# pixeli99/SVD_Xtend

Measured on NVIDIA H100. Metric: SVD UNet train-step frames/sec @ 14x320x512 bf16, higher is better.
Workload: dtype bf16

## Files before the change

include/svd_xtend_b200.h:

```cpp
#ifndef SVD_XTEND_B200_H_
#define SVD_XTEND_B200_H_

#include <stdint.h>

#ifdef __cplusplus
extern "C" {
#endif

#define SVDX_OK 0
#define SVDX_E_BADARG (-1)
#define SVDX_E_CUDA (-2)
#define SVDX_E_NODRIVER (-3)

#define SVDX_MAX_TAPS 27

#define SVDX_A_ROWS 0
#define SVDX_A_CONV2D 1

#define SVDX_OUT_BF16 0
#define SVDX_OUT_F32 1
#define SVDX_OUT_F32_ATOMIC 2

typedef struct SvdxTapGemm {
  const void* a;
// ... 23 lines not shown
  int64_t ldrb;
  const void* res1;
  int64_t ldr1;
  const void* res2;
  int64_t ldr2;
  const float* scales;
  void* pre;
  int64_t ldpre;
  float* gn_sum;
  int64_t gn_ld;
  int32_t gn_rows;
  const void* gnb_x;
  int64_t gnb_ldx;
  const void* gnb_x2;
  int64_t gnb_ldx2;
  int32_t gnb_c1;
  const float* gnb_ab;
  float* gnb_sum;
  int32_t gnb_rows;
  int32_t gnb_silu;
  int32_t interleave;
  int32_t phase_h, phase_w;
  int32_t act;
} SvdxTapGemm;

#define SVDX_ACT_NONE 0
#define SVDX_ACT_GELU 1
#define SVDX_ACT_QUICK_GELU 2

int svdx_tapgemm(const SvdxTapGemm* desc, void* stream);

int svdx_splitk_epilogue(float* ws, int64_t ldw, void* out, int64_t ldo, int64_t rows, int32_t cols, const float* bias,
                         const float* rowbias, int32_t rowbias_div, int64_t ldrb, const void* res1, int64_t ldr1,
                         const void* res2, int64_t ldr2, const float* scales, void* stream);

int svdx_num_sms(void);
int svdx_enable_peer_access(int32_t peer_device);
int svdx_ipc_export(const void* ptr, void* handle64_out, int64_t* offset_out);
int svdx_ipc_import(const void* handle64, int64_t offset, void** ptr_out);
int svdx_struct_size(int which);
const char* svdx_last_error(void);

int svdx_groupnorm_sums(const void* x, int64_t ldx, int32_t C1, const void* x2, int64_t ldx2, int32_t C2,
                        int32_t outer, int32_t rows, float* sums, int64_t ld, void* stream);
int svdx_groupnorm_apply_fused(const void* x, int64_t ldx, int32_t C1, const void* x2, int64_t ldx2, int32_t C2,
                               int32_t outer, int32_t rows, int32_t num_groups, float eps,
                               const float* csum1, int64_t ldc1, const float* csum2, int64_t ldc2,
                               float* mean, float* rstd, const float* gamma, const float* beta,
                               int32_t fuse_silu, void* y, int64_t ldy, float* ab_out, void* stream);
int svdx_groupnorm_bwd_sums(const void* x, int64_t ldx, int32_t C1, const void* x2, int64_t ldx2, int32_t C2,
                            const void* dy, int64_t lddy, int32_t outer, int32_t rows, const float* ab, int32_t fuse_silu,
// ... 146 lines not shown
```

svd_xtend_b200/_lib.py:

```python
from __future__ import annotations

import ctypes as C
import os
from pathlib import Path

PKG = Path(__file__).resolve().parent
LIB_PATH = Path(os.environ["SVDX_LIB"]) if os.environ.get("SVDX_LIB") else PKG / "lib" / "libsvdx_b200.so"

SVDX_MAX_TAPS = 27
SVDX_CLIP_MAX_TAPS = 63
A_ROWS, A_CONV2D = 0, 1
OUT_BF16, OUT_F32, OUT_F32_ATOMIC = 0, 1, 2
ACT_NONE, ACT_GELU, ACT_QUICK_GELU = 0, 1, 2

c_void_p, c_int, c_i64, c_float = C.c_void_p, C.c_int32, C.c_int64, C.c_float


class SvdxTapGemm(C.Structure):
    _fields_ = [
        ("a", c_void_p), ("lda", c_i64), ("a_mode", c_int), ("a_major_mn", c_int),
        ("rows_per_group", c_int), ("groups", c_int),
        ("W", c_int), ("H", c_int), ("nimg", c_int),
        ("num_taps", c_int),
        ("tap_d0", c_int * SVDX_MAX_TAPS), ("tap_d1", c_int * SVDX_MAX_TAPS), ("tap_d2", c_int * SVDX_MAX_TAPS),
        ("b", c_void_p), ("ldb", c_i64), ("b_major_mn", c_int), ("b_mode", c_int),
        ("M", c_int), ("N", c_int), ("K", c_int),
        ("block_n", c_int), ("split_k", c_int),
        ("out", c_void_p), ("ldo", c_i64), ("out_dtype", c_int), ("geglu", c_int),
        ("bias", c_void_p), ("rowbias", c_void_p), ("rowbias_div", c_int), ("ldrb", c_i64),
        ("res1", c_void_p), ("ldr1", c_i64), ("res2", c_void_p), ("ldr2", c_i64),
        ("scales", c_void_p), ("pre", c_void_p), ("ldpre", c_i64),
        ("gn_sum", c_void_p), ("gn_ld", c_i64), ("gn_rows", c_int),
        ("gnb_x", c_void_p), ("gnb_ldx", c_i64), ("gnb_x2", c_void_p), ("gnb_ldx2", c_i64), ("gnb_c1", c_int),
        ("gnb_ab", c_void_p), ("gnb_sum", c_void_p), ("gnb_rows", c_int), ("gnb_silu", c_int),
        ("interleave", c_int), ("phase_h", c_int), ("phase_w", c_int),
        ("act", c_int),
    ]


class SvdxAttn(C.Structure):
    _fields_ = [
        ("q", c_void_p), ("k", c_void_p), ("v", c_void_p), ("o", c_void_p),
        ("ldq", c_i64), ("ldk", c_i64), ("ldv", c_i64), ("ldo", c_i64),
        ("nseq", c_int), ("heads", c_int), ("S", c_int), ("inner", c_int),
        ("outer_stride", c_i64), ("inner_stride", c_i64), ("tok_stride", c_i64),
        ("scale", c_float), ("lse", c_void_p),
        ("dout", c_void_p), ("lddo", c_i64),
        ("dq", c_void_p), ("dk", c_void_p), ("dv", c_void_p),
        ("lddq", c_i64), ("lddk", c_i64), ("lddv", c_i64),
        ("delta", c_void_p),
    ]


_PROTOS = {
    "svdx_tapgemm": [C.POINTER(SvdxTapGemm), c_void_p],
    "svdx_splitk_epilogue": [c_void_p, c_i64, c_void_p, c_i64, c_i64, c_int, c_void_p, c_void_p, c_int, c_i64, c_void_p, c_i64,
                             c_void_p, c_i64, c_void_p, c_void_p],
    "svdx_num_sms": [],
    "svdx_enable_peer_access": [c_int],
# ... 126 lines not shown
```

svd_xtend_b200/csrc/common.cuh:

```cuda
#pragma once
#include <cuda.h>
#include <cuda_bf16.h>
#include <cuda_runtime.h>
#include <stdint.h>
#include <stdio.h>

#include "wgmma.cuh"

namespace svdx {

typedef __nv_bfloat16 bf16;

#define SVDX_DEVINL __device__ __forceinline__

#ifndef SVDX_WAIT_TIMEOUT_CYCLES
#define SVDX_WAIT_TIMEOUT_CYCLES (4000000000ll)
#endif

SVDX_DEVINL uint32_t smem_u32(const void* p) { return (uint32_t)__cvta_generic_to_shared(p); }

SVDX_DEVINL uint32_t lane_id() { return threadIdx.x & 31; }

SVDX_DEVINL bool elect_one() {
  uint32_t pred = 0;
// ... 93 lines not shown
               ::"l"(reinterpret_cast<uint64_t>(m)), "r"(src), "r"(c0), "r"(c1), "r"(c2)
               : "memory");
}
SVDX_DEVINL void bulk_commit() { asm volatile("cp.async.bulk.commit_group;" ::: "memory"); }
template <int N>
SVDX_DEVINL void bulk_wait_read() { asm volatile("cp.async.bulk.wait_group.read %0;" ::"n"(N) : "memory"); }
template <int N>
SVDX_DEVINL void bulk_wait() { asm volatile("cp.async.bulk.wait_group %0;" ::"n"(N) : "memory"); }
SVDX_DEVINL void st_shared_v4(uint32_t addr, uint32_t a, uint32_t b, uint32_t c, uint32_t d) {
  asm volatile("st.shared.v4.b32 [%0], {%1, %2, %3, %4};" ::"r"(addr), "r"(a), "r"(b), "r"(c), "r"(d) : "memory");
}

SVDX_DEVINL void wgmma_fence() { asm volatile("wgmma.fence.sync.aligned;" ::: "memory"); }
SVDX_DEVINL void wgmma_commit() { asm volatile("wgmma.commit_group.sync.aligned;" ::: "memory"); }
template <int N>
SVDX_DEVINL void wgmma_wait() { asm volatile("wgmma.wait_group.sync.aligned %0;" ::"n"(N) : "memory"); }
template <int R>
SVDX_DEVINL void reg_fence(float (&d)[R]) {
#pragma unroll
  for (int i = 0; i < R; ++i) asm volatile("" : "+f"(d[i])::"memory");
}

SVDX_DEVINL void named_bar_sync(int id, int nthreads) { asm volatile("bar.sync %0, %1;" ::"r"(id), "r"(nthreads) : "memory"); }

SVDX_DEVINL uint64_t make_smem_desc_sw128(uint32_t saddr, uint32_t lbo_bytes, uint32_t sbo_bytes) {
  uint64_t d = 0;
  d |= (uint64_t)((saddr & 0x3FFFF) >> 4);
  d |= (uint64_t)((lbo_bytes >> 4) & 0x3FFF) << 16;
  d |= (uint64_t)((sbo_bytes >> 4) & 0x3FFF) << 32;
  d |= (uint64_t)1 << 62;
  return d;
}

SVDX_DEVINL float silu_f(float x) { return __fdividef(x, 1.0f + __expf(-x)); }
SVDX_DEVINL float silu_grad_f(float x) {
  const float s = __fdividef(1.0f, 1.0f + __expf(-x));
  return s * fmaf(x, 1.0f - s, 1.0f);
}
#define SVDX_HDINL __host__ __device__ __forceinline__
SVDX_HDINL float gelu_tail_log2(float ax) {
  float p = -1.92123457e-06f;
  p = fmaf(p, ax, 6.32884985e-05f);
  p = fmaf(p, ax, -0.000943420862f);
  p = fmaf(p, ax, 0.0085562719f);
  p = fmaf(p, ax, -0.0540522821f);
  p = fmaf(p, ax, -0.458381772f);
// ... 45 lines not shown
```

svd_xtend_b200/csrc/tapgemm.cu:

```cuda
#include "tapgemm_common.cuh"

namespace svdx {

struct Ring {
  uint32_t sA, sB, bar_full, bar_empty;
  int stage;
  uint32_t phase;
};
template <int BN, int TA, int TB, int STG>
__device__ __forceinline__ void tile_mainloop(float (&acc)[BN / 2], int kb0, int kb1, Ring& rg, int wg) {
#pragma unroll
  for (int i = 0; i < BN / 2; ++i) acc[i] = 0.f;
  const int lane = threadIdx.x & 31;
  const uint32_t astep = TA ? (2048 >> 4) : (32 >> 4), bstep = TB ? (2048 >> 4) : (32 >> 4);
  int prev_stage = -1;
  for (int kb = kb0; kb < kb1; ++kb) {
    mbar_wait_mma(rg.bar_full + 8 * rg.stage, rg.phase);
    const uint32_t aaddr = rg.sA + rg.stage * A_STAGE_BYTES + wg * 8192;
    const uint32_t baddr = rg.sB + rg.stage * B_STAGE_BYTES;
    const uint64_t ad0 = make_smem_desc_sw128(aaddr, 8192, 1024);
    const uint64_t bd0 = make_smem_desc_sw128(baddr, 8192, 1024);
    wgmma_fence();
#pragma unroll
    for (int j = 0; j < BLOCK_K / 16; ++j) {
      const uint32_t accumulate = (kb > kb0 || j > 0) ? 1u : 0u;
      if constexpr (BN == 32) wgmma_ss_n32<TA, TB>(acc, ad0 + j * astep, bd0 + j * bstep, accumulate);
      else if constexpr (BN == 64) wgmma_ss_n64<TA, TB>(acc, ad0 + j * astep, bd0 + j * bstep, accumulate);
      else if constexpr (BN == 96) wgmma_ss_n96<TA, TB>(acc, ad0 + j * astep, bd0 + j * bstep, accumulate);
      else if constexpr (BN == 128) wgmma_ss_n128<TA, TB>(acc, ad0 + j * astep, bd0 + j * bstep, accumulate);
      else wgmma_ss_n160<TA, TB>(acc, ad0 + j * astep, bd0 + j * bstep, accumulate);
    }
    wgmma_commit();
    wgmma_wait<1>();
    reg_fence(acc);
    if (prev_stage >= 0) {
      __syncwarp();
      if (lane == 0) mbar_arrive(rg.bar_empty + 8 * prev_stage);
    }
    prev_stage = rg.stage;
    if (++rg.stage == STG) { rg.stage = 0; rg.phase ^= 1; }
  }
  wgmma_wait<0>();
  reg_fence(acc);
  __syncwarp();
  if (lane == 0 && prev_stage >= 0) mbar_arrive(rg.bar_empty + 8 * prev_stage);
}

template <int BN, int TA, int TB>
SVDX_DEVINL void tile_parked_bn(int kb0, int kb1, Ring& rg, uint32_t sAcc, int wg) {
  float acc[BN / 2];
  tile_mainloop<BN, TA, TB, STAGES_PARKED>(acc, kb0, kb1, rg, wg);
  const int lane = threadIdx.x & 31;
  const int r0 = wg * 64 + ((threadIdx.x >> 5) & 3) * 16 + (lane >> 2);
// ... 30 lines not shown
SVDX_DEVINL void tile_regs(const TapGemmKParams& p, int kb0, int kb1, Ring& rg, int wg, PairStage& ps, const EpiTile& t, int lane,
                           float s_acc, float s_r1, float s_r2) {
  if constexpr (EPI == EPI_GEGLU) {
    if (p.block_n == 64) tile_regs_bn<EPI, 64, 0>(p, kb0, kb1, rg, wg, ps, t, lane, s_acc, s_r1, s_r2);
    else tile_regs_bn<EPI, 128, 0>(p, kb0, kb1, rg, wg, ps, t, lane, s_acc, s_r1, s_r2);
  } else {
    if constexpr (EPI == EPI_FAST) {
      if (p.b_mn) {
        if (p.block_n == 64) tile_regs_bn<EPI, 64, 1>(p, kb0, kb1, rg, wg, ps, t, lane, s_acc, s_r1, s_r2);
        else tile_regs_bn<EPI, 128, 1>(p, kb0, kb1, rg, wg, ps, t, lane, s_acc, s_r1, s_r2);
        return;
      }
    }
    switch (p.block_n) {
      case 32: tile_regs_bn<EPI, 32, 0>(p, kb0, kb1, rg, wg, ps, t, lane, s_acc, s_r1, s_r2); break;
      case 64: tile_regs_bn<EPI, 64, 0>(p, kb0, kb1, rg, wg, ps, t, lane, s_acc, s_r1, s_r2); break;
      case 96: tile_regs_bn<EPI, 96, 0>(p, kb0, kb1, rg, wg, ps, t, lane, s_acc, s_r1, s_r2); break;
      case 128: tile_regs_bn<EPI, 128, 0>(p, kb0, kb1, rg, wg, ps, t, lane, s_acc, s_r1, s_r2); break;
      default: tile_regs_bn<EPI, 160, 0>(p, kb0, kb1, rg, wg, ps, t, lane, s_acc, s_r1, s_r2); break;
    }
  }
}

template <int BN, int TA, int TB>
SVDX_DEVINL void tile_f32_bn(const TapGemmKParams& p, int kb0, int kb1, Ring& rg, int wg, EpiStage& st, const EpiTile& t, int sub, int lane,
                             float s_acc) {
  float acc[BN / 2];
  tile_mainloop<BN, TA, TB, STAGES_REGS>(acc, kb0, kb1, rg, wg);
  epilogue_f32<BN>(p, acc, st, t, sub, lane, s_acc);
}

template <int TA>
SVDX_DEVINL void tile_f32(const TapGemmKParams& p, int kb0, int kb1, Ring& rg, int wg, EpiStage& st, const EpiTile& t, int sub, int lane,
                          float s_acc) {
  if (p.b_mn) {
    if (p.block_n == 64) tile_f32_bn<64, TA, 1>(p, kb0, kb1, rg, wg, st, t, sub, lane, s_acc);
    else tile_f32_bn<128, TA, 1>(p, kb0, kb1, rg, wg, st, t, sub, lane, s_acc);
    return;
  }
  switch (p.block_n) {
    case 32: tile_f32_bn<32, TA, 0>(p, kb0, kb1, rg, wg, st, t, sub, lane, s_acc); break;
    case 64: tile_f32_bn<64, TA, 0>(p, kb0, kb1, rg, wg, st, t, sub, lane, s_acc); break;
    case 96: tile_f32_bn<96, TA, 0>(p, kb0, kb1, rg, wg, st, t, sub, lane, s_acc); break;
    case 128: tile_f32_bn<128, TA, 0>(p, kb0, kb1, rg, wg, st, t, sub, lane, s_acc); break;
    default: tile_f32_bn<160, TA, 0>(p, kb0, kb1, rg, wg, st, t, sub, lane, s_acc); break;
  }
}

template <int EPI>
__global__ void __launch_bounds__(NUM_THREADS, 1) tapgemm_kernel(const __grid_constant__ TapGemmKParams p) {
  constexpr bool PARKED = EPI == EPI_GENERIC;
  constexpr int STAGES = PARKED ? STAGES_PARKED : STAGES_REGS;
  extern __shared__ uint8_t smem_raw[];
  const uint32_t smem_base = (smem_u32(smem_raw) + 1023u) & ~1023u;
  const uint32_t sA = smem_base;
  const uint32_t sB = smem_base + STAGES * A_STAGE_BYTES;
  const uint32_t sAcc = sB + STAGES * B_STAGE_BYTES;
  const uint32_t sEpi = sAcc + (PARKED ? ACC_BYTES : 0);
  const uint32_t sBar = sEpi + NUM_EPI_WARPS * EPI_STAGE_BYTES;
  const uint32_t bar_full = sBar;
  const uint32_t bar_empty = sBar + 8 * STAGES;

  const int warp = threadIdx.x >> 5;
  const int lane = threadIdx.x & 31;

  if (warp == PRODUCER_WARP && lane == 0) {
    prefetch_tmap(&p.tma);
    prefetch_tmap(&p.tmb);
    for (int i = 0; i < STAGES; ++i) {
      mbar_init(bar_full + 8 * i, 1);
      mbar_init(bar_empty + 8 * i, NUM_EPI_WARPS);
    }
    fence_barrier_init();
  }
  __syncthreads();

  const int total_tiles = p.m_tiles * p.n_tiles * p.split_k;
  const int b_bytes = p.block_n * BLOCK_K * 2;

  if (warp == PRODUCER_WARP) {
    const bool conv_par = (p.a_mode == SVDX_A_CONV2D) && !p.a_mn && !p.b_mn && !p.geglu && !p.wtiles && !p.im2col && (BLOCK_M / p.W) <= 32;
    if (conv_par) {
      int stage = 0;
      uint32_t phase = 0;
      for (int tile = blockIdx.x; tile < total_tiles; tile += gridDim.x) {
        const int nt = tile % p.n_tiles;
        const int mt = (tile / p.n_tiles) % p.m_tiles;
        const int ks = tile / (p.n_tiles * p.m_tiles);
        const int kb0 = ks * p.kb_per_split;
        const int kb1 = min(kb0 + p.kb_per_split, p.kb_total);
        const int n0 = nt * p.block_n;
        ConvBox bx;
        conv_tile_boxes(p, mt, lane, bx);
        const CUtensorMap* amap = bx.lg == 0 ? &p.tma : &p.tma_bh[bx.lg - 1];
        int tap = kb0 / p.kb_per_tap;
        int kci = kb0 - tap * p.kb_per_tap;
        for (int kb = kb0; kb < kb1; ++kb) {
          const uint32_t full = bar_full + 8 * stage;
          if (lane == 0) {
            mbar_wait_mma(bar_empty + 8 * stage, phase ^ 1);
            mbar_expect_tx(full, A_STAGE_BYTES + b_bytes);
// ... 138 lines not shown
                  tma_load_4d(&p.tmb, full, dB + j * 8192 + i * p.W * 128, n0 + 64 * j, dw, row - n * p.H + dh, nn);
                }
              }
            }
          } else if (p.b_mn && p.b_mode == 2) {
            const int g = kb / p.kb_per_group;
            const int k0 = (kb - g * p.kb_per_group) * BLOCK_K;
            for (int j = 0; j < p.block_n / 64; ++j)
              tma_load_3d(&p.tmb, full, dB + j * 8192, n0 + 64 * j, k0 + p.tap_d0[0], g);
          } else if (p.b_mn) {
            for (int j = 0; j < p.block_n / 64; ++j)
              tma_load_2d(&p.tmb, full, dB + j * 8192, n0 + 64 * j, kb * BLOCK_K);
          } else if (p.geglu) {
            const int h = p.block_n / 2;
            tma_load_2d(&p.tmb, full, dB, tap * p.K + kc, n0);
            tma_load_2d(&p.tmb, full, dB + h * 128, tap * p.K + kc, p.N / 2 + n0);
          } else {
            tma_load_2d(&p.tmb, full, dB, tap * p.K + kc, n0);
          }
          if (++stage == STAGES) { stage = 0; phase ^= 1; }
        }
      }
    }
  } else {
    const int wg = warp >> 2;
    const int q = PARKED ? (warp & 3) : (warp >> 1);
    const int half = PARKED ? (warp >> 2) : (warp & 1);
    Ring rg{sA, sB, bar_full, bar_empty, 0, 0u};
    float s_acc = 1.f, s_r1 = 1.f, s_r2 = 1.f;
    if (p.scales) { s_acc = p.scales[0]; s_r1 = p.scales[1]; s_r2 = p.scales[2]; }
    const int n_out_total = p.geglu ? p.N / 2 : p.N;
    const int bn_out = p.geglu ? p.block_n / 2 : p.block_n;
    EpiStage st;
    st.base = sEpi + warp * EPI_STAGE_BYTES;
    st.off = 0;
    PairStage ps{sEpi + q * 2 * EPI_STAGE_BYTES, 2 + q, half, 0u};
    const uint32_t t_base = sAcc + (uint32_t)((q * 32 + lane) * ACC_LD) * 4u;
    for (int tile = blockIdx.x; tile < total_tiles; tile += gridDim.x) {
      const int nt = tile % p.n_tiles;
      const int mt = (tile / p.n_tiles) % p.m_tiles;
      const int ks = tile / (p.n_tiles * p.m_tiles);
      const int kb0 = ks * p.kb_per_split;
      const int kb1 = min(kb0 + p.kb_per_split, p.kb_total);
      const int n0 = nt * bn_out;
      long long m;
      bool row_ok;
// ... 277 lines not shown
    if (d->act != SVDX_ACT_GELU && d->act != SVDX_ACT_QUICK_GELU) return svdx_fail(SVDX_E_BADARG, "tapgemm: act must be SVDX_ACT_GELU or SVDX_ACT_QUICK_GELU");
    if (p.epi_mode != EPI_FAST || p.rowbias || p.split_k > 1 || p.gn_sum)
      return svdx_fail(SVDX_E_BADARG, "tapgemm: act needs the plain bf16 TMA-store epilogue (bias only: no rowbias / residual / scales / "
                                      "GEGLU / split-K / gn_sum / gnb sums / interleave; N %% 32 == 0, aligned rows)");
    p.act = d->act;
    p.epi_mode = EPI_FAST_ACT;
  }
  if (d->b_major_mn && p.epi_mode != EPI_GENERIC && p.epi_mode != EPI_F32 && (p.epi_mode != EPI_FAST || p.gn_sum))
    return svdx_fail(SVDX_E_BADARG, "tapgemm: MN-major B takes the plain epilogue only (no gn_sum / gnb sums / act)");
  if (wide320 && p.epi_mode != EPI_FAST && p.epi_mode != EPI_RES && p.epi_mode != EPI_FAST_GNB && p.epi_mode != EPI_FAST_IL && p.epi_mode != EPI_FAST_ACT)
    return svdx_fail(SVDX_E_BADARG, "tapgemm: block_n 320 needs a bf16 output through the TMA-store epilogues (N % 320 == 0, aligned rows)");
  if (p.gn_sum) {
    if (p.epi_mode != EPI_FAST && p.epi_mode != EPI_RES && p.epi_mode != EPI_FAST_IL)
      return svdx_fail(SVDX_E_BADARG, "tapgemm: gn_sum needs a bf16 output through the TMA-store epilogues (N % 32 == 0, aligned rows), no split-K / GEGLU");
    if (p.gn_rows <= 0 || p.gn_ld < n_out || (p.gn_ld & 1) || (reinterpret_cast<uintptr_t>(p.gn_sum) & 7))
      return svdx_fail(SVDX_E_BADARG, "tapgemm: gn_sum needs gn_rows > 0, even gn_ld >= N, 8-byte aligned buffer");
  }
  if (d->out_dtype == SVDX_OUT_BF16 && ((d->ldo % 8) || (reinterpret_cast<uintptr_t>(d->out) & 15))) return svdx_fail(SVDX_E_BADARG, "tapgemm: out alignment");
  if (d->out_dtype != SVDX_OUT_BF16 && ((d->ldo % 4) || (reinterpret_cast<uintptr_t>(d->out) & 15))) return svdx_fail(SVDX_E_BADARG, "tapgemm: out alignment");
  if (d->res1 && ((d->ldr1 % 8) || (reinterpret_cast<uintptr_t>(d->res1) & 15))) return svdx_fail(SVDX_E_BADARG, "tapgemm: res1 alignment");
  if (d->res2 && ((d->ldr2 % 8) || (reinterpret_cast<uintptr_t>(d->res2) & 15))) return svdx_fail(SVDX_E_BADARG, "tapgemm: res2 alignment");
  if (d->pre && ((d->ldpre % 8) || (reinterpret_cast<uintptr_t>(d->pre) & 15))) return svdx_fail(SVDX_E_BADARG, "tapgemm: pre alignment");

  return SVDX_OK;
}

static constexpr int kernel_smem(int epi) { return epi == EPI_GENERIC ? smem_bytes(STAGES_PARKED, true) : smem_bytes(STAGES_REGS, false); }

template <int EPI>
static cudaError_t set_smem() {
  return cudaFuncSetAttribute(tapgemm_kernel<EPI>, cudaFuncAttributeMaxDynamicSharedMemorySize, kernel_smem(EPI));
}
template <int EPI>
static void launch(int grid, cudaStream_t stream, const TapGemmKParams& p) {
  tapgemm_kernel<EPI><<<grid, NUM_THREADS, kernel_smem(EPI), stream>>>(p);
}

extern "C" int svdx_tapgemm(const SvdxTapGemm* d, void* stream_v) {
  cudaStream_t stream = reinterpret_cast<cudaStream_t>(stream_v);
  TapGemmKParams p;
  int rc = svdx_tapgemm_fill(d, p);
  if (rc) return rc;
  static bool attr_done[SVDX_MAX_DEVICES] = {false};
  const int slot = svdx_device_slot();
  if (!attr_done[slot]) {
    cudaError_t e = set_smem<EPI_GENERIC>();
    if (e == cudaSuccess) e = set_smem<EPI_FAST>();
    if (e == cudaSuccess) e = set_smem<EPI_GEGLU>();
    if (e == cudaSuccess) e = set_smem<EPI_RES>();
    if (e == cudaSuccess) e = set_smem<EPI_FAST_GN>();
    if (e == cudaSuccess) e = set_smem<EPI_RES_GN>();
    if (e == cudaSuccess) e = set_smem<EPI_FAST_GNB>();
    if (e == cudaSuccess) e = set_smem<EPI_FAST_IL>();
    if (e == cudaSuccess) e = set_smem<EPI_FAST_IL_GN>();
    if (e == cudaSuccess) e = set_smem<EPI_FAST_ACT>();
    if (e == cudaSuccess) e = set_smem<EPI_F32>();
    if (e != cudaSuccess) return svdx_fail_cuda(e, "tapgemm: set smem attribute");
    attr_done[slot] = true;
  }
  const int total_tiles = p.m_tiles * p.n_tiles * p.split_k;
  int grid = svdx_num_sms();
  if (grid > total_tiles) grid = total_tiles;
  if (p.epi_mode == EPI_F32) launch<EPI_F32>(grid, stream, p);
  else if (p.epi_mode == EPI_FAST_ACT) launch<EPI_FAST_ACT>(grid, stream, p);
  else if (p.epi_mode == EPI_FAST_IL && p.gn_sum) launch<EPI_FAST_IL_GN>(grid, stream, p);
  else if (p.epi_mode == EPI_FAST_IL) launch<EPI_FAST_IL>(grid, stream, p);
  else if (p.epi_mode == EPI_FAST_GNB) launch<EPI_FAST_GNB>(grid, stream, p);
  else if (p.epi_mode == EPI_FAST && p.gn_sum) launch<EPI_FAST_GN>(grid, stream, p);
  else if (p.epi_mode == EPI_RES && p.gn_sum) launch<EPI_RES_GN>(grid, stream, p);
  else if (p.epi_mode == EPI_FAST) launch<EPI_FAST>(grid, stream, p);
  else if (p.epi_mode == EPI_GEGLU) launch<EPI_GEGLU>(grid, stream, p);
  else if (p.epi_mode == EPI_RES) launch<EPI_RES>(grid, stream, p);
  else launch<EPI_GENERIC>(grid, stream, p);
  cudaError_t e = cudaGetLastError();
  if (e != cudaSuccess) return svdx_fail_cuda(e, "tapgemm: launch");
  return SVDX_OK;
}
```

svd_xtend_b200/csrc/tapgemm_common.cuh:

```cuda
#pragma once
#include "common.cuh"
#include "../../include/svd_xtend_b200.h"
#include "host_util.h"

namespace svdx {

constexpr int BLOCK_M = 128;
constexpr int BLOCK_K = 64;
constexpr int MAX_BN = 160;
constexpr int A_STAGE_BYTES = BLOCK_M * BLOCK_K * 2;
constexpr int B_STAGE_BYTES = MAX_BN * BLOCK_K * 2;
constexpr int NUM_EPI_WARPS = 8;
constexpr int PRODUCER_WARP = NUM_EPI_WARPS;
constexpr int NUM_THREADS = 32 * NUM_EPI_WARPS + 32;
constexpr int ACC_LD = MAX_BN + 4;
constexpr int ACC_BYTES = BLOCK_M * ACC_LD * 4;
constexpr int EPI_STAGE_BYTES = 4096;
constexpr int STAGES_PARKED = 3;
constexpr int STAGES_REGS = 5;
constexpr int smem_bytes(int stages, bool parked) {
  return 1024 + stages * (A_STAGE_BYTES + B_STAGE_BYTES) + (parked ? ACC_BYTES : 0) + NUM_EPI_WARPS * EPI_STAGE_BYTES + 256;
}
static_assert(smem_bytes(STAGES_PARKED, true) <= 227 * 1024, "tapgemm shared memory exceeds the 227 KB a block may use");
static_assert(smem_bytes(STAGES_REGS, false) <= 227 * 1024, "tapgemm shared memory exceeds the 227 KB a block may use");
static_assert(16 * STAGES_REGS <= 256, "ring barriers must fit their 256-byte region");
static_assert((ACC_BYTES % 1024) == 0 && (B_STAGE_BYTES % 1024) == 0, "staging buffers must stay 1024-byte aligned");

struct __align__(64) TapGemmKParams {
  CUtensorMap tma;
  CUtensorMap tmb;
  CUtensorMap tma_bh[4];
  int max_bh_log2;
  int a_mode, a_mn, b_mn, b_mode, kb_per_group;
  int rows_per_group, groups, tiles_per_group;
  int W, H, nimg;
  int wtiles;
  int im2col;
// ... 11 lines not shown
  const bf16* res1;
  long long ldr1;
  const bf16* res2;
  long long ldr2;
  const float* scales;
  bf16* pre;
  long long ldpre;
  CUtensorMap tmo;
  CUtensorMap tmo16;
  CUtensorMap tmpre;
  float* gn_sum;
  long long gn_ld;
  int gn_rows;
  const bf16* gnb_x;
  long long gnb_ldx;
  const bf16* gnb_x2;
  long long gnb_ldx2;
  int gnb_c1;
  const float* gnb_ab;
  float* gnb_sum;
  int gnb_rows, gnb_silu;
  int tma_store;
  int epi_mode;
  int probe;
  int interleave;
  int act;
  bf16* il_out;
};


SVDX_DEVINL void acc_ld32(uint32_t row, int col, uint32_t (&r)[32]) {
  const uint32_t a = row + col * 4;
#pragma unroll
  for (int k = 0; k < 8; ++k)
    asm volatile("ld.shared.v4.b32 {%0, %1, %2, %3}, [%4];" : "=r"(r[4 * k]), "=r"(r[4 * k + 1]), "=r"(r[4 * k + 2]), "=r"(r[4 * k + 3])
                 : "r"(a + 16 * k));
}

SVDX_DEVINL void tile_row(const TapGemmKParams& p, int mt, int r, long long& m, bool& row_ok) {
  if (p.a_mode == SVDX_A_ROWS && !p.a_mn) {
    const int g = mt / p.tiles_per_group;
    const int t = mt - g * p.tiles_per_group;
    const int rin = t * BLOCK_M + r;
    row_ok = rin < p.rows_per_group;
    m = (long long)g * p.rows_per_group + rin;
  } else {
// ... 646 lines not shown
```

svd_xtend_b200/raw.py:

```python
from __future__ import annotations

import ctypes as C
import functools
import math
import os
from typing import Optional, Sequence

import numpy as np
import torch

from . import _lib
from ._lib import ACT_GELU, ACT_NONE, ACT_QUICK_GELU, A_CONV2D, A_ROWS, OUT_BF16, OUT_F32, OUT_F32_ATOMIC, SvdxAttn, SvdxTapGemm, load

bf16 = torch.bfloat16

_DTYPE_CODE = {torch.float32: 0, torch.bfloat16: 1, torch.float16: 2}


def dtype_code(t: torch.Tensor, what: str) -> int:
    try:
        return _DTYPE_CODE[t.dtype]
    except KeyError:
        raise TypeError(f"svd_xtend_b200: {what} has dtype {t.dtype}; supported: float32, bfloat16, float16") from None

LAUNCHES = [0]
_KERNELS_PER_CALL = {"svdx_groupnorm_apply_fused": 1, "svdx_attention_bwd": 3, "svdx_adamw_graph": 2, "svdx_adamw_p2p": 2,
                     "svdx_adamw_graph_ema": 2, "svdx_adamw_p2p_ema": 2, "svdx_ema_multi": 2, "svdx_adamw8bit": 2,
                     "svdx_adamw8bit_ema": 2, "svdx_adamw_graph_mul": 2, "svdx_adamw_graph_ema_mul": 2, "svdx_adamw8bit_mul": 2,
                     "svdx_adamw8bit_ema_mul": 2, "svdx_adamw_p2p_mul": 2, "svdx_adamw_p2p_ema_mul": 2, "svdx_grad_sumsq": 2,
                     "svdx_grad_sumsq_p2p": 2, "svdx_adamw8bit_p2p": 2}


def check(rc: int, what: str = "") -> None:
    LAUNCHES[0] += _KERNELS_PER_CALL.get(what, 1)
    _lib.check(rc, what)
# ... 63 lines not shown


def choose_block_n(M: int, n_out: int, geglu: bool = False, mn_major: bool = False) -> int:
    sms = num_sms()
    if mn_major:
        best, best_cost = None, None
        m_tiles = (M + 127) // 128
        for bn in (128, 64):
            cost = m_tiles * ((n_out + bn - 1) // bn) * max(bn / 2.0, 32.0 + bn / 4.0)
            if best_cost is None or cost < best_cost - 1e-9:
                best, best_cost = bn, cost
        return best
    cands = [64, 32] if geglu else [160, 128, 96, 64, 32]
    best, best_cost = None, None
    for bn in cands:
        if n_out % bn and n_out > bn:
            continue
        cost = _tile_cost(M, n_out, bn, geglu, sms)
        if best_cost is None or cost < best_cost * 0.98:
            best, best_cost = bn, cost
    if best is None:
        best = pick_block_n(n_out, False)
    return 2 * best if geglu else best


WIDE_TILE = os.environ.get("SVDX_WIDE", "1") != "0"
WIDE_MIN_K = int(os.environ.get("SVDX_WIDE_MIN_K", "960"))


def _wide_tile_ok(M, N, k_total, out, ldo, geglu, a_mn, b_mn, b_mode, split_k, out_dtype, bias, rowbias) -> bool:
    if not WIDE_TILE or geglu or a_mn or b_mn or b_mode != 0 or split_k != 1 or N % 320 or N % 256 == 0 or M < 512 or k_total < WIDE_MIN_K:
        return False
    if out.dtype != bf16 or (out_dtype is not None and out_dtype != OUT_BF16):
        return False
    ld = ldo if ldo is not None else out.stride(0)
    if ld % 8 or out.data_ptr() % 16:
        return False
    if bias is not None and bias.data_ptr() % 16:
        return False
    if rowbias is not None and (rowbias.data_ptr() % 16 or rowbias.stride(0) % 4):
        return False
    return True


_WGRAD_SM_BYTES_PER_CLK = 34.0
_WGRAD_L2_BYTES_PER_CLK = 4500.0
# ... 43 lines not shown
    conv_whn: Optional[Sequence[int]] = None,
    lda: Optional[int] = None,
    ldb: Optional[int] = None,
    ldo: Optional[int] = None,
    a_mn: bool = False,
    b_mn: bool = False,
    b_mode: int = 0,
    block_n: Optional[int] = None,
    split_k: int = 1,
    out_dtype: Optional[int] = None,
    geglu: bool = False,
    bias: Optional[torch.Tensor] = None,
    rowbias: Optional[torch.Tensor] = None,
    rowbias_div: int = 1,
    res1: Optional[torch.Tensor] = None,
    res2: Optional[torch.Tensor] = None,
    scales: Optional[torch.Tensor] = None,
    pre: Optional[torch.Tensor] = None,
    gn_sum: Optional[torch.Tensor] = None,
    gn_rows: int = 0,
    gnb: Optional[dict] = None,
    phase: Optional[Sequence[int]] = None,
    act: int = ACT_NONE,
) -> torch.Tensor:
    family = "conv" if (mode == A_CONV2D or len(taps) > 1 or b_mode != 0) else "linear"
    if _fam(family, 2.0 * M * N * K * len(taps)):
        return out
    if SHAPE_LOG is not None:
        SHAPE_LOG.append(dict(M=M, N=N, K=K, taps=len(taps), conv2d=int(mode == A_CONV2D), geglu=int(geglu), a_mn=int(a_mn), b_mode=b_mode,
                              split_k=split_k, block_n=block_n, f32out=int(out.dtype != bf16), bias=int(bias is not None),
                              rowbias=int(rowbias is not None), res=int(res1 is not None) + int(res2 is not None),
                              scales=int(scales is not None), pre=int(pre is not None),
                              launch=dict(M=M, N=N, K=K, mode=mode, taps=[[int(v) for v in t] for t in taps], rows_per_group=rows_per_group,
                                          groups=groups, conv_whn=None if conv_whn is None else [int(v) for v in conv_whn], lda=lda, ldb=ldb,
                                          ldo=ldo, a_mn=bool(a_mn), b_mn=bool(b_mn), b_mode=b_mode, block_n=block_n, split_k=split_k,
                                          out_dtype=out_dtype, geglu=bool(geglu), rowbias_div=rowbias_div, gn_rows=gn_rows,
                                          phase=None if phase is None else [int(v) for v in phase], act=int(act),
                                          gnb=None if gnb is None else dict(rows=int(gnb["rows"]), silu=bool(gnb["silu"])),
                                          tensors={k: _layout(t) for k, t in (
                                              ("a", a), ("b", b), ("out", out), ("bias", bias), ("rowbias", rowbias), ("res1", res1),
                                              ("res2", res2), ("scales", scales), ("pre", pre), ("gn_sum", gn_sum),
                                              ("gnb_x", None if gnb is None else gnb["x"]), ("gnb_x2", None if gnb is None else gnb.get("x2")),
                                              ("gnb_ab", None if gnb is None else gnb.get("ab")), ("gnb_sum", None if gnb is None else gnb["sum"]))
                                              if t is not None})))
    d = SvdxTapGemm()
    assert a.dtype == bf16 and b.dtype == bf16
    d.a = a.data_ptr()
    d.lda = lda if lda is not None else _rowmajor(a, "a")
    d.a_mode = mode
    d.a_major_mn = int(a_mn)
    d.rows_per_group = rows_per_group if rows_per_group is not None else M
    d.groups = groups
    if conv_whn is not None:
        d.W, d.H, d.nimg = conv_whn
    d.num_taps = len(taps)
    for i, t in enumerate(taps):
        d.tap_d0[i], d.tap_d1[i], d.tap_d2[i] = int(t[0]), int(t[1]), int(t[2])
    d.b = b.data_ptr()
    d.ldb = ldb if ldb is not None else _rowmajor(b, "b")
    d.b_major_mn = int(b_mn)
    d.b_mode = b_mode
    d.M, d.N, d.K = M, N, K
    n_out = N // 2 if geglu else N
    if block_n is None:
        block_n = choose_block_n(M, n_out, geglu, b_mn)
        if _wide_tile_ok(M, N, K * len(taps), out, ldo, geglu, a_mn, b_mn, b_mode, split_k, out_dtype, bias, rowbias):
            block_n = 320
    d.block_n = block_n
    d.split_k = split_k
    d.out = out.data_ptr()
    d.ldo = ldo if ldo is not None else _rowmajor(out, "out")
    if out_dtype is None:
        out_dtype = OUT_BF16 if out.dtype == bf16 else OUT_F32
    d.out_dtype = out_dtype
    d.geglu = int(geglu)
    if bias is not None:
        assert bias.dtype == torch.float32
        d.bias = bias.data_ptr()
    if rowbias is not None:
        assert rowbias.dtype == torch.float32
        d.rowbias = rowbias.data_ptr()
        d.rowbias_div = rowbias_div
        d.ldrb = _rowmajor(rowbias, "rowbias")
    if res1 is not None:
        assert res1.dtype == bf16
        d.res1 = res1.data_ptr()
        d.ldr1 = _rowmajor(res1, "res1")
    if res2 is not None:
        assert res2.dtype == bf16
        d.res2 = res2.data_ptr()
        d.ldr2 = _rowmajor(res2, "res2")
# ... 710 lines not shown
```

Measured before the change: 159.4.

## Add ping-pong warpgroup schedule to tap GEMM with cost-model selection

```diff
diff --git a/include/svd_xtend_b200.h b/include/svd_xtend_b200.h
--- a/include/svd_xtend_b200.h
+++ b/include/svd_xtend_b200.h
@@ -69,11 +69,14 @@
   int32_t interleave;
   int32_t phase_h, phase_w;
   int32_t act;
+  int32_t schedule;
 } SvdxTapGemm;
 
 #define SVDX_ACT_NONE 0
 #define SVDX_ACT_GELU 1
 #define SVDX_ACT_QUICK_GELU 2
+#define SVDX_SCHED_COOP 0
+#define SVDX_SCHED_PINGPONG 1
 
 int svdx_tapgemm(const SvdxTapGemm* desc, void* stream);
 
diff --git a/svd_xtend_b200/_lib.py b/svd_xtend_b200/_lib.py
--- a/svd_xtend_b200/_lib.py
+++ b/svd_xtend_b200/_lib.py
@@ -12,6 +12,7 @@
 A_ROWS, A_CONV2D = 0, 1
 OUT_BF16, OUT_F32, OUT_F32_ATOMIC = 0, 1, 2
 ACT_NONE, ACT_GELU, ACT_QUICK_GELU = 0, 1, 2
+SCHED_COOP, SCHED_PINGPONG = 0, 1
 
 c_void_p, c_int, c_i64, c_float = C.c_void_p, C.c_int32, C.c_int64, C.c_float
 
@@ -34,7 +35,7 @@
         ("gnb_x", c_void_p), ("gnb_ldx", c_i64), ("gnb_x2", c_void_p), ("gnb_ldx2", c_i64), ("gnb_c1", c_int),
         ("gnb_ab", c_void_p), ("gnb_sum", c_void_p), ("gnb_rows", c_int), ("gnb_silu", c_int),
         ("interleave", c_int), ("phase_h", c_int), ("phase_w", c_int),
-        ("act", c_int),
+        ("act", c_int), ("schedule", c_int),
     ]
 
 
diff --git a/svd_xtend_b200/csrc/common.cuh b/svd_xtend_b200/csrc/common.cuh
--- a/svd_xtend_b200/csrc/common.cuh
+++ b/svd_xtend_b200/csrc/common.cuh
@@ -139,6 +139,7 @@
 }
 
 SVDX_DEVINL void named_bar_sync(int id, int nthreads) { asm volatile("bar.sync %0, %1;" ::"r"(id), "r"(nthreads) : "memory"); }
+SVDX_DEVINL void named_bar_arrive(int id, int nthreads) { asm volatile("bar.arrive %0, %1;" ::"r"(id), "r"(nthreads) : "memory"); }
 
 SVDX_DEVINL uint64_t make_smem_desc_sw128(uint32_t saddr, uint32_t lbo_bytes, uint32_t sbo_bytes) {
   uint64_t d = 0;
diff --git a/svd_xtend_b200/csrc/tapgemm.cu b/svd_xtend_b200/csrc/tapgemm.cu
--- a/svd_xtend_b200/csrc/tapgemm.cu
+++ b/svd_xtend_b200/csrc/tapgemm.cu
@@ -7,6 +7,15 @@
   int stage;
   uint32_t phase;
 };
+template <int BN, int TA, int TB>
+__device__ __forceinline__ void wgmma_bn(float (&acc)[BN / 2], uint64_t ad, uint64_t bd, uint32_t accumulate) {
+  if constexpr (BN == 32) wgmma_ss_n32<TA, TB>(acc, ad, bd, accumulate);
+  else if constexpr (BN == 64) wgmma_ss_n64<TA, TB>(acc, ad, bd, accumulate);
+  else if constexpr (BN == 96) wgmma_ss_n96<TA, TB>(acc, ad, bd, accumulate);
+  else if constexpr (BN == 128) wgmma_ss_n128<TA, TB>(acc, ad, bd, accumulate);
+  else wgmma_ss_n160<TA, TB>(acc, ad, bd, accumulate);
+}
+
 template <int BN, int TA, int TB, int STG>
 __device__ __forceinline__ void tile_mainloop(float (&acc)[BN / 2], int kb0, int kb1, Ring& rg, int wg) {
 #pragma unroll
@@ -24,11 +33,7 @@
 #pragma unroll
     for (int j = 0; j < BLOCK_K / 16; ++j) {
       const uint32_t accumulate = (kb > kb0 || j > 0) ? 1u : 0u;
-      if constexpr (BN == 32) wgmma_ss_n32<TA, TB>(acc, ad0 + j * astep, bd0 + j * bstep, accumulate);
-      else if constexpr (BN == 64) wgmma_ss_n64<TA, TB>(acc, ad0 + j * astep, bd0 + j * bstep, accumulate);
-      else if constexpr (BN == 96) wgmma_ss_n96<TA, TB>(acc, ad0 + j * astep, bd0 + j * bstep, accumulate);
-      else if constexpr (BN == 128) wgmma_ss_n128<TA, TB>(acc, ad0 + j * astep, bd0 + j * bstep, accumulate);
-      else wgmma_ss_n160<TA, TB>(acc, ad0 + j * astep, bd0 + j * bstep, accumulate);
+      wgmma_bn<BN, TA, TB>(acc, ad0 + j * astep, bd0 + j * bstep, accumulate);
     }
     wgmma_commit();
     wgmma_wait<1>();
@@ -105,6 +110,97 @@
   }
 }
 
+constexpr int PP_BAR = 6;
+
+SVDX_DEVINL int tile_kblocks(const TapGemmKParams& p, int tile) {
+  const int kb0 = (tile / (p.n_tiles * p.m_tiles)) * p.kb_per_split;
+  return min(kb0 + p.kb_per_split, p.kb_total) - kb0;
+}
+
+SVDX_DEVINL void ring_skip(Ring& rg, int kblocks, int stages) {
+  const int s = rg.stage + kblocks;
+  rg.phase ^= (uint32_t)((s / stages) & 1);
+  rg.stage = s % stages;
+}
+
+template <int BN, int STG>
+__device__ __forceinline__ void tile_mainloop_pp(float (&acc0)[BN / 2], float (&acc1)[BN / 2], int kb0, int kb1, Ring& rg, int handoff) {
+#pragma unroll
+  for (int i = 0; i < BN / 2; ++i) { acc0[i] = 0.f; acc1[i] = 0.f; }
+  const int lane = threadIdx.x & 31;
+  int prev_stage = -1;
+  for (int kb = kb0; kb < kb1; ++kb) {
+    mbar_wait_mma(rg.bar_full + 8 * rg.stage, rg.phase);
+    const uint32_t aaddr = rg.sA + rg.stage * A_STAGE_BYTES;
+    const uint64_t ad0 = make_smem_desc_sw128(aaddr, 8192, 1024);
+    const uint64_t ad1 = make_smem_desc_sw128(aaddr + 8192, 8192, 1024);
+    const uint64_t bd0 = make_smem_desc_sw128(rg.sB + rg.stage * B_STAGE_BYTES, 8192, 1024);
+    wgmma_fence();
+#pragma unroll
+    for (int j = 0; j < BLOCK_K / 16; ++j) {
+      const uint32_t accumulate = (kb > kb0 || j > 0) ? 1u : 0u;
+      wgmma_bn<BN, 0, 0>(acc0, ad0 + j * 2, bd0 + j * 2, accumulate);
+      wgmma_bn<BN, 0, 0>(acc1, ad1 + j * 2, bd0 + j * 2, accumulate);
+    }
+    wgmma_commit();
+    wgmma_wait<1>();
+    reg_fence(acc0);
+    reg_fence(acc1);
+    if (prev_stage >= 0) {
+      __syncwarp();
+      if (lane == 0) mbar_arrive(rg.bar_empty + 8 * prev_stage);
+    }
+    prev_stage = rg.stage;
+    if (++rg.stage == STG) { rg.stage = 0; rg.phase ^= 1; }
+  }
+  if (handoff >= 0) named_bar_arrive(handoff, 2 * 128);
+  wgmma_wait<0>();
+  reg_fence(acc0);
+  reg_fence(acc1);
+  __syncwarp();
+  if (lane == 0 && prev_stage >= 0) mbar_arrive(rg.bar_empty + 8 * prev_stage);
+}
+
+template <int EPI, int BN>
+SVDX_DEVINL void tile_regs_pp_bn(const TapGemmKParams& p, int kb0, int kb1, Ring& rg, int handoff, PairStage& ps, const EpiTile (&t)[2],
+                                 int lane, float s_acc, float s_r1, float s_r2) {
+  float acc0[BN / 2], acc1[BN / 2];
+  tile_mainloop_pp<BN, STAGES_REGS>(acc0, acc1, kb0, kb1, rg, handoff);
+  epilogue_regs<EPI, BN>(p, acc0, ps, t[0], lane, s_acc, s_r1, s_r2);
+  epilogue_regs<EPI, BN>(p, acc1, ps, t[1], lane, s_acc, s_r1, s_r2);
+}
+
+template <int EPI>
+SVDX_DEVINL void tile_regs_pp(const TapGemmKParams& p, int kb0, int kb1, Ring& rg, int handoff, PairStage& ps, const EpiTile (&t)[2], int lane,
+                              float s_acc, float s_r1, float s_r2) {
+  if constexpr (EPI != EPI_GEGLU) {
+    if (p.block_n == 96) {
+      tile_regs_pp_bn<EPI, 96>(p, kb0, kb1, rg, handoff, ps, t, lane, s_acc, s_r1, s_r2);
+      return;
+    }
+  }
+  if (p.block_n == 64) tile_regs_pp_bn<EPI, 64>(p, kb0, kb1, rg, handoff, ps, t, lane, s_acc, s_r1, s_r2);
+  else tile_regs_pp_bn<EPI, 128>(p, kb0, kb1, rg, handoff, ps, t, lane, s_acc, s_r1, s_r2);
+}
+
+SVDX_DEVINL void quarter_tile(const TapGemmKParams& p, int mt, int q, int sub, int lane, int n0, int n_out_total, EpiTile& et) {
+  et.n0 = n0;
+  et.n_out_total = n_out_total;
+  if (p.a_mode == SVDX_A_ROWS && !p.a_mn) {
+    et.grp = mt / p.tiles_per_group;
+    et.row0 = (mt - et.grp * p.tiles_per_group) * BLOCK_M + q * 32;
+    et.m0 = (long long)et.grp * p.rows_per_group + et.row0;
+    et.valid_rows = max(0, min(32, p.rows_per_group - et.row0));
+  } else {
+    et.grp = 0;
+    et.row0 = mt * BLOCK_M + q * 32;
+    et.m0 = et.row0;
+    et.valid_rows = max(0, min(32, p.M - et.row0));
+  }
+#pragma unroll
+  for (int h = 0; h < 2; ++h) tile_row(p, mt, q * 32 + sub * 16 + (lane >> 2) + 8 * h, et.m[h], et.ok[h]);
+}
+
 template <int BN, int TA, int TB>
 SVDX_DEVINL void tile_f32_bn(const TapGemmKParams& p, int kb0, int kb1, Ring& rg, int wg, EpiStage& st, const EpiTile& t, int sub, int lane,
                              float s_acc) {
@@ -130,8 +226,10 @@
   }
 }
 
-template <int EPI>
-__global__ void __launch_bounds__(NUM_THREADS, 1) tapgemm_kernel(const __grid_constant__ TapGemmKParams p) {
+template <int EPI, bool PP>
+__global__ void __launch_bounds__(PP ? NUM_THREADS_PP : NUM_THREADS, 1) tapgemm_kernel(const __grid_constant__ TapGemmKParams p) {
+  static_assert(!PP || EPI == EPI_FAST || EPI == EPI_FAST_GN || EPI == EPI_FAST_GNB || EPI == EPI_RES || EPI == EPI_RES_GN || EPI == EPI_GEGLU,
+                "ping-pong runs the bf16 register epilogues only");
   constexpr bool PARKED = EPI == EPI_GENERIC;
   constexpr int STAGES = PARKED ? STAGES_PARKED : STAGES_REGS;
   extern __shared__ uint8_t smem_raw[];
@@ -152,7 +250,7 @@
     prefetch_tmap(&p.tmb);
     for (int i = 0; i < STAGES; ++i) {
       mbar_init(bar_full + 8 * i, 1);
-      mbar_init(bar_empty + 8 * i, NUM_EPI_WARPS);
+      mbar_init(bar_empty + 8 * i, PP ? NUM_EPI_WARPS / 2 : NUM_EPI_WARPS);
     }
     fence_barrier_init();
   }
@@ -160,6 +258,14 @@
 
   const int total_tiles = p.m_tiles * p.n_tiles * p.split_k;
   const int b_bytes = p.block_n * BLOCK_K * 2;
+  if constexpr (PP) {
+    if (warp >= NUM_EPI_WARPS) {
+      asm volatile("setmaxnreg.dec.sync.aligned.u32 %0;" ::"n"(PP_PRODUCER_REGS));
+      if (warp != PRODUCER_WARP) return;
+    } else {
+      asm volatile("setmaxnreg.inc.sync.aligned.u32 %0;" ::"n"(PP_CONSUMER_REGS));
+    }
+  }
 
   if (warp == PRODUCER_WARP) {
     const bool conv_par = (p.a_mode == SVDX_A_CONV2D) && !p.a_mn && !p.b_mn && !p.geglu && !p.wtiles && !p.im2col && (BLOCK_M / p.W) <= 32;
@@ -344,6 +450,35 @@
         }
       }
     }
+  } else if constexpr (PP) {
+    const int wg = warp >> 2;
+    const int sub = warp & 1;
+    const int pq = (warp & 3) >> 1;
+    Ring rg{sA, sB, bar_full, bar_empty, 0, 0u};
+    float s_acc = 1.f, s_r1 = 1.f, s_r2 = 1.f;
+    if (p.scales) { s_acc = p.scales[0]; s_r1 = p.scales[1]; s_r2 = p.scales[2]; }
+    const int n_out_total = p.geglu ? p.N / 2 : p.N;
+    const int bn_out = p.geglu ? p.block_n / 2 : p.block_n;
+    PairStage ps{sEpi + (warp >> 1) * 2 * EPI_STAGE_BYTES, 2 + (warp >> 1), sub, 0u};
+    for (int tile = blockIdx.x + wg * gridDim.x, i = wg; tile < total_tiles; tile += 2 * gridDim.x, i += 2) {
+      if (i > 0) ring_skip(rg, tile_kblocks(p, tile - gridDim.x), STAGES);
+      const int nt = tile % p.n_tiles;
+      const int mt = (tile / p.n_tiles) % p.m_tiles;
+      const int kb0 = (tile / (p.n_tiles * p.m_tiles)) * p.kb_per_split;
+      const int kb1 = min(kb0 + p.kb_per_split, p.kb_total);
+      const int n0 = nt * bn_out;
+      EpiTile et[2];
+#pragma unroll
+      for (int h = 0; h < 2; ++h) {
+        quarter_tile(p, mt, pq + 2 * h, sub, lane, n0, n_out_total, et[h]);
+        if constexpr (EPI == EPI_RES || EPI == EPI_RES_GN || EPI == EPI_FAST_GNB)
+          prefetch_epilogue_operands(p, EPI, et[h].m0, et[h].valid_rows, n0, bn_out, n_out_total, lane, sub);
+      }
+      if (i > 0) named_bar_sync(PP_BAR + wg, 2 * 128);
+      const int handoff = tile + gridDim.x < total_tiles ? PP_BAR + (wg ^ 1) : -1;
+      tile_regs_pp<EPI>(p, kb0, kb1, rg, handoff, ps, et, lane, s_acc, s_r1, s_r2);
+    }
+    if (lane == 0) bulk_wait<0>();
   } else {
     const int wg = warp >> 2;
     const int q = PARKED ? (warp & 3) : (warp >> 1);
@@ -667,18 +802,27 @@
   if (d->res2 && ((d->ldr2 % 8) || (reinterpret_cast<uintptr_t>(d->res2) & 15))) return svdx_fail(SVDX_E_BADARG, "tapgemm: res2 alignment");
   if (d->pre && ((d->ldpre % 8) || (reinterpret_cast<uintptr_t>(d->pre) & 15))) return svdx_fail(SVDX_E_BADARG, "tapgemm: pre alignment");
 
+  if (d->schedule != SVDX_SCHED_COOP && d->schedule != SVDX_SCHED_PINGPONG) return svdx_fail(SVDX_E_BADARG, "tapgemm: schedule");
+  if (d->schedule == SVDX_SCHED_PINGPONG) {
+    const bool epi_ok = p.epi_mode == EPI_FAST || p.epi_mode == EPI_FAST_GNB || p.epi_mode == EPI_RES || p.epi_mode == EPI_GEGLU;
+    const bool bn_ok = d->geglu ? (block_n == 64 || block_n == 128) : (block_n == 64 || block_n == 96 || block_n == 128);
+    if (!epi_ok || !bn_ok || wide320 || d->b_major_mn || p.split_k > 1)
+      return svdx_fail(SVDX_E_BADARG, "tapgemm: the ping-pong schedule needs a bf16 register epilogue without interleave / act (N %% 32 == 0, "
+                                      "aligned rows), K-major B, no split-K and block_n 64 / 96 / 128 (GEGLU: 64 / 128)");
+    p.pingpong = 1;
+  }
   return SVDX_OK;
 }
 
 static constexpr int kernel_smem(int epi) { return epi == EPI_GENERIC ? smem_bytes(STAGES_PARKED, true) : smem_bytes(STAGES_REGS, false); }
 
-template <int EPI>
+template <int EPI, bool PP = false>
 static cudaError_t set_smem() {
-  return cudaFuncSetAttribute(tapgemm_kernel<EPI>, cudaFuncAttributeMaxDynamicSharedMemorySize, kernel_smem(EPI));
-}
-template <int EPI>
+  return cudaFuncSetAttribute(tapgemm_kernel<EPI, PP>, cudaFuncAttributeMaxDynamicSharedMemorySize, kernel_smem(EPI));
+}
+template <int EPI, bool PP = false>
 static void launch(int grid, cudaStream_t stream, const TapGemmKParams& p) {
-  tapgemm_kernel<EPI><<<grid, NUM_THREADS, kernel_smem(EPI), stream>>>(p);
+  tapgemm_kernel<EPI, PP><<<grid, PP ? NUM_THREADS_PP : NUM_THREADS, kernel_smem(EPI), stream>>>(p);
 }
 
 extern "C" int svdx_tapgemm(const SvdxTapGemm* d, void* stream_v) {
@@ -700,13 +844,26 @@
     if (e == cudaSuccess) e = set_smem<EPI_FAST_IL_GN>();
     if (e == cudaSuccess) e = set_smem<EPI_FAST_ACT>();
     if (e == cudaSuccess) e = set_smem<EPI_F32>();
+    if (e == cudaSuccess) e = set_smem<EPI_FAST, true>();
+    if (e == cudaSuccess) e = set_smem<EPI_GEGLU, true>();
+    if (e == cudaSuccess) e = set_smem<EPI_RES, true>();
+    if (e == cudaSuccess) e = set_smem<EPI_FAST_GN, true>();
+    if (e == cudaSuccess) e = set_smem<EPI_RES_GN, true>();
+    if (e == cudaSuccess) e = set_smem<EPI_FAST_GNB, true>();
     if (e != cudaSuccess) return svdx_fail_cuda(e, "tapgemm: set smem attribute");
     attr_done[slot] = true;
   }
   const int total_tiles = p.m_tiles * p.n_tiles * p.split_k;
   int grid = svdx_num_sms();
   if (grid > total_tiles) grid = total_tiles;
-  if (p.epi_mode == EPI_F32) launch<EPI_F32>(grid, stream, p);
+  if (p.pingpong) {
+    if (p.epi_mode == EPI_FAST_GNB) launch<EPI_FAST_GNB, true>(grid, stream, p);
+    else if (p.epi_mode == EPI_FAST && p.gn_sum) launch<EPI_FAST_GN, true>(grid, stream, p);
+    else if (p.epi_mode == EPI_RES && p.gn_sum) launch<EPI_RES_GN, true>(grid, stream, p);
+    else if (p.epi_mode == EPI_FAST) launch<EPI_FAST, true>(grid, stream, p);
+    else if (p.epi_mode == EPI_GEGLU) launch<EPI_GEGLU, true>(grid, stream, p);
+    else launch<EPI_RES, true>(grid, stream, p);
+  } else if (p.epi_mode == EPI_F32) launch<EPI_F32>(grid, stream, p);
   else if (p.epi_mode == EPI_FAST_ACT) launch<EPI_FAST_ACT>(grid, stream, p);
   else if (p.epi_mode == EPI_FAST_IL && p.gn_sum) launch<EPI_FAST_IL_GN>(grid, stream, p);
   else if (p.epi_mode == EPI_FAST_IL) launch<EPI_FAST_IL>(grid, stream, p);
diff --git a/svd_xtend_b200/csrc/tapgemm_common.cuh b/svd_xtend_b200/csrc/tapgemm_common.cuh
--- a/svd_xtend_b200/csrc/tapgemm_common.cuh
+++ b/svd_xtend_b200/csrc/tapgemm_common.cuh
@@ -13,6 +13,9 @@
 constexpr int NUM_EPI_WARPS = 8;
 constexpr int PRODUCER_WARP = NUM_EPI_WARPS;
 constexpr int NUM_THREADS = 32 * NUM_EPI_WARPS + 32;
+constexpr int NUM_THREADS_PP = 32 * NUM_EPI_WARPS + 128;
+constexpr int PP_PRODUCER_REGS = 40, PP_CONSUMER_REGS = 232;
+static_assert(128 * PP_PRODUCER_REGS + 256 * PP_CONSUMER_REGS <= NUM_THREADS_PP * 168, "ping-pong register split");
 constexpr int ACC_LD = MAX_BN + 4;
 constexpr int ACC_BYTES = BLOCK_M * ACC_LD * 4;
 constexpr int EPI_STAGE_BYTES = 4096;
@@ -70,6 +73,7 @@
   int gnb_rows, gnb_silu;
   int tma_store;
   int epi_mode;
+  int pingpong;
   int probe;
   int interleave;
   int act;
diff --git a/svd_xtend_b200/raw.py b/svd_xtend_b200/raw.py
--- a/svd_xtend_b200/raw.py
+++ b/svd_xtend_b200/raw.py
@@ -10,7 +10,7 @@
 import torch
 
 from . import _lib
-from ._lib import ACT_GELU, ACT_NONE, ACT_QUICK_GELU, A_CONV2D, A_ROWS, OUT_BF16, OUT_F32, OUT_F32_ATOMIC, SvdxAttn, SvdxTapGemm, load
+from ._lib import ACT_GELU, ACT_NONE, ACT_QUICK_GELU, A_CONV2D, A_ROWS, OUT_BF16, OUT_F32, OUT_F32_ATOMIC, SCHED_COOP, SCHED_PINGPONG, SvdxAttn, SvdxTapGemm, load
 
 bf16 = torch.bfloat16
 
@@ -120,6 +120,68 @@
     if best is None:
         best = pick_block_n(n_out, False)
     return 2 * best if geglu else best
+
+
+PINGPONG = int(os.environ.get("SVDX_PINGPONG", "1"))
+_EPI_CLK = {"fast": 150.0, "fast_gn": 250.0, "res": 175.0, "res_gn": 350.0, "gnb": 375.0, "geglu": 300.0, "geglu_pre": 450.0}
+
+
+def _sched_cost(M: int, n_out: int, bn_out: int, geglu: bool, kb: int, epi: str, pingpong: bool, sms: int) -> float:
+    bn = 2 * bn_out if geglu else bn_out
+    ctas = ((M + 127) // 128) * ((n_out + bn_out - 1) // bn_out)
+    active = min(ctas, sms)
+    per_kb = max(4 * max(bn / 2.0, 32.0 + bn / 4.0), (16384 + 128 * bn) * active / _L2_BYTES_PER_CLK)
+    ml = kb * per_kb
+    e = _EPI_CLK[epi] * (bn_out / 32.0)
+    t = -(-ctas // sms)
+    if not pingpong:
+        return t * (ml + e)
+    return ml + (t - 1) * max(ml, (ml + 2 * e) / 2) + 2 * e
+
+
+def choose_schedule(M: int, n_out: int, kb: int, geglu: bool, epi: str, mode: int = PINGPONG):
+    coop = choose_block_n(M, n_out, geglu)
+    if mode == 0:
+        return coop, SCHED_COOP
+    sms = num_sms()
+    best, best_cost = None, None
+    for bn in ((64, 32) if geglu else (128, 96, 64)):
+        cost = _sched_cost(M, n_out, bn, geglu, kb, epi, True, sms)
+        if best_cost is None or cost < best_cost * 0.98:
+            best, best_cost = bn, cost
+    pp = 2 * best if geglu else best
+    if mode == 2:
+        return pp, SCHED_PINGPONG
+    coop_out = coop // 2 if geglu else coop
+    if ((M + 127) // 128) * ((n_out + best - 1) // best) <= sms:
+        return coop, SCHED_COOP
+    if best_cost < _sched_cost(M, n_out, coop_out, geglu, kb, epi, False, sms):
+        return pp, SCHED_PINGPONG
+    return coop, SCHED_COOP
+
+
+def _pingpong_epi(N, out, ldo, geglu, a_mn, b_mn, b_mode, split_k, out_dtype, bias, rowbias, res, pre, gn_sum, gnb, phase, act):
+    if a_mn or b_mn or b_mode != 0 or split_k != 1 or phase is not None or act:
+        return None
+    if os.environ.get("SVDX_TMA_STORE", "1") != "1" or os.environ.get("SVDX_EPI_PROBE", "0") != "0":
+        return None
+    if out.dtype != bf16 or (out_dtype is not None and out_dtype != OUT_BF16):
+        return None
+    n_out = N // 2 if geglu else N
+    ld = ldo if ldo is not None else out.stride(0)
+    if n_out % 32 or ld % 8 or out.data_ptr() % 16:
+        return None
+    if bias is not None and bias.data_ptr() % 16:
+        return None
+    if rowbias is not None and (rowbias.data_ptr() % 16 or rowbias.stride(0) % 4):
+        return None
+    if geglu:
+        if pre is not None and ((N // 2) % 32 or pre.stride(0) % 8 or pre.data_ptr() % 16):
+            return None
+        return "geglu" if pre is None else "geglu_pre"
+    if gnb is not None:
+        return "gnb"
+    return ("res" if res else "fast") + ("_gn" if gn_sum is not None else "")
 
 
 WIDE_TILE = os.environ.get("SVDX_WIDE", "1") != "0"
@@ -209,6 +271,7 @@
     gnb: Optional[dict] = None,
     phase: Optional[Sequence[int]] = None,
     act: int = ACT_NONE,
+    schedule: Optional[int] = None,
 ) -> torch.Tensor:
     family = "conv" if (mode == A_CONV2D or len(taps) > 1 or b_mode != 0) else "linear"
     if _fam(family, 2.0 * M * N * K * len(taps)):
@@ -224,6 +287,7 @@
                                           out_dtype=out_dtype, geglu=bool(geglu), rowbias_div=rowbias_div, gn_rows=gn_rows,
                                           phase=None if phase is None else [int(v) for v in phase], act=int(act),
                                           gnb=None if gnb is None else dict(rows=int(gnb["rows"]), silu=bool(gnb["silu"])),
+                                          schedule=schedule,
                                           tensors={k: _layout(t) for k, t in (
                                               ("a", a), ("b", b), ("out", out), ("bias", bias), ("rowbias", rowbias), ("res1", res1),
                                               ("res2", res2), ("scales", scales), ("pre", pre), ("gn_sum", gn_sum),
@@ -249,11 +313,19 @@
     d.b_mode = b_mode
     d.M, d.N, d.K = M, N, K
     n_out = N // 2 if geglu else N
+    sched = SCHED_COOP if schedule is None else schedule
     if block_n is None:
         block_n = choose_block_n(M, n_out, geglu, b_mn)
-        if _wide_tile_ok(M, N, K * len(taps), out, ldo, geglu, a_mn, b_mn, b_mode, split_k, out_dtype, bias, rowbias):
+        sched = SCHED_COOP
+        mode = PINGPONG if schedule is None else (0 if schedule == SCHED_COOP else 2)
+        epi = None if mode == 0 else _pingpong_epi(N, out, ldo, geglu, a_mn, b_mn, b_mode, split_k, out_dtype, bias, rowbias,
+                                                   res1 is not None or res2 is not None or scales is not None, pre, gn_sum, gnb, phase, act)
+        if epi is not None:
+            block_n, sched = choose_schedule(M, n_out, -(-K // 64) * len(taps), geglu, epi, mode)
+        if sched == SCHED_COOP and _wide_tile_ok(M, N, K * len(taps), out, ldo, geglu, a_mn, b_mn, b_mode, split_k, out_dtype, bias, rowbias):
             block_n = 320
     d.block_n = block_n
+    d.schedule = sched
     d.split_k = split_k
     d.out = out.data_ptr()
     d.ldo = ldo if ldo is not None else _rowmajor(out, "out")
```

Result: faster. 163.0 (median of 6 runs) (+2.2%).
